# turian/inverse-audio-synthesis

Measured on AMD Instinct MI355X. Metric: audio-seconds rendered+lossed/sec (whole node), batch=128 4s@44.1kHz, higher is better.
Workload: dtype f32; 1 GPU; BASELINE configs[1]: torchsynth-style Voice render + PQMF(3) analysis + mel-L1 loss, batch 128 x 4 s @ 44100 Hz per GPU; batch_per_gpu=128, samples_per_voice=176400, launch=hipgraph, streams=5, pipelined=True

## Files before the change

inverse-audio-synthesis_amd/csrc/voice_ctrl_kernels.hip:

```cpp
#define IAS_CTL_NO_LIBM
#include "voice_math.h"
#include "wave_ops.h"
#include "voice_table.h"

#define CS_THREADS 256
#define CS_WAVES (CS_THREADS / 64)
#define CS_KERNEL __global__ __launch_bounds__(CS_THREADS) __attribute__((amdgpu_num_vgpr(28)))

__constant__ IasParamRange c_cs_table[IAS_NPARAMS] = IAS_PARAM_TABLE_INIT;
__device__ const double g_cs_tab[IAS_CTL_TAB_DOUBLES] = IAS_CTL_TAB_INIT;

__device__ __forceinline__ void cs_stage_table(double* s_tab) {
  for (int i = threadIdx.x; i < IAS_CTL_TAB_DOUBLES; i += CS_THREADS) s_tab[i] = g_cs_tab[i];
}
__device__ __forceinline__ float cs_mapped(const float* __restrict__ params01, int b, int idx, const double* s_tab) {
  const IasParamRange r = c_cs_table[idx];
  return ias_map_param(params01[(size_t)b * IAS_NPARAMS + idx], (float)r.lo, (float)r.span, (float)r.curve, r.symmetric, s_tab);
}
__device__ __forceinline__ int cs_adsr_base(int a) {
  switch (a) {
    case 0: return IAS_P_ADSR_1_ATTACK;
    case 1: return IAS_P_ADSR_2_ATTACK;
    case 2: return IAS_P_LFO_1_AMP_ADSR_ATTACK;
    case 3: return IAS_P_LFO_2_AMP_ADSR_ATTACK;
    case 4: return IAS_P_LFO_1_RATE_ADSR_ATTACK;
    default: return IAS_P_LFO_2_RATE_ADSR_ATTACK;
  }
}

CS_KERNEL void voice_env_slim_kernel(const float* __restrict__ params01, float* __restrict__ sig, int Tc, float control_rate) {
  __shared__ __attribute__((aligned(16))) double s_tab[IAS_CTL_TAB_DOUBLES];
  __shared__ float s_p[8];
  const int a = blockIdx.x, b = blockIdx.y, tid = threadIdx.x;
  cs_stage_table(s_tab);
  __syncthreads();
  if (tid < 5) s_p[tid] = cs_mapped(params01, b, cs_adsr_base(a) + tid, s_tab);
  if (tid == 5) s_p[5] = cs_mapped(params01, b, IAS_P_KEYBOARD_DURATION, s_tab);
  __syncthreads();
  IasAdsr e;
  e.attack = s_p[0]; e.decay = s_p[1]; e.sustain = s_p[2]; e.release = s_p[3]; e.alpha = s_p[4];
  const float note_on = s_p[5], eps = (float)IAS_EPS;
  if (tid == 0) s_p[6] = ias_adsr_heads(e, note_on, control_rate, eps, s_tab).decay_head;
  if (tid == 64) s_p[7] = ias_adsr_heads(e, note_on, control_rate, eps, s_tab).release_head;
  __syncthreads();
  IasAdsrHeads heads;
  heads.decay_head = s_p[6]; heads.release_head = s_p[7];
  float* out = sig + ((size_t)b * 8 + a) * Tc;
  for (int t = tid; t < Tc; t += CS_THREADS) out[t] = ias_adsr_headed(t, e, note_on, control_rate, eps, heads, s_tab);
}

CS_KERNEL void voice_lfo_slim_kernel(const float* __restrict__ params01, float* __restrict__ sig,
                                     float* __restrict__ dbg ,
                                     int Tc, float control_rate) {
  extern __shared__ __attribute__((aligned(16))) double cs_smem[];
  double* s_tab = cs_smem;
  double* s_sum = s_tab + IAS_CTL_TAB_DOUBLES;
  __shared__ double s_wtot[CS_WAVES];
  __shared__ float s_q[8];
  __shared__ float s_mode[8];
  const int l = blockIdx.x, b = blockIdx.y, tid = threadIdx.x, lane = tid & 63, wave = tid >> 6;
  const int qbase = (l == 0) ? IAS_P_LFO_1_FREQUENCY : IAS_P_LFO_2_FREQUENCY;
  cs_stage_table(s_tab);
  __syncthreads();
  if (tid < 8) s_q[tid] = cs_mapped(params01, b, qbase + tid, s_tab);
  __syncthreads();
  if (tid < 5) s_mode[tid] = ias_pow_ctl(s_q[3 + tid], IAS_LFO_EXPONENT_F, s_tab);
  const float freq = s_q[0], depth = s_q[1], phi = s_q[2];
  const float* rate_env = sig + ((size_t)b * 8 + 4 + l) * Tc;
  const float* amp_env = sig + ((size_t)b * 8 + 2 + l) * Tc;

  const int per_wave = ((Tc + CS_WAVES - 1) / CS_WAVES + 63) / 64 * 64;
  const int t_begin = min(wave * per_wave, Tc), t_end = min(t_begin + per_wave, Tc);
  double carry = 0.0;
  for (int t0 = t_begin; t0 < t_end; t0 += 64) {
    const int t = t0 + lane;
    double inc = 0.0;
    if (t < t_end) inc = (double)ias_lfo_inc(freq, depth, rate_env[t], control_rate);
    const double sc = wave_incl_scan(inc, lane) + carry;
    carry = __shfl(sc, 63, 64);
    if (t < t_end) s_sum[t] = sc;
  }
  if (lane == 0) s_wtot[wave] = carry;
  __syncthreads();
  double base = 0.0;
  for (int w = 0; w < wave; ++w) base += s_wtot[w];
  float mode[5];
  {
    const float sm = (float)((double)s_mode[0] + (double)s_mode[1] + (double)s_mode[2] + (double)s_mode[3] + (double)s_mode[4]);
#pragma unroll
    for (int k = 0; k < 5; ++k) mode[k] = ias_div(s_mode[k], sm);
  }
  float* out = sig + ((size_t)b * 8 + 6 + l) * Tc;
  for (int t = t_begin + lane; t < t_end; t += 64) {
    const double ph = base + s_sum[t];
    const float arg = ias_add((float)ph, phi);
    const float o = ias_mul(ias_lfo_shape_mix(arg, mode, s_tab), amp_env[t]);
    out[t] = o;
    if (dbg != nullptr) {
      dbg[((size_t)b * 10 + 6 + l) * Tc + t] = arg;
      dbg[((size_t)b * 10 + 8 + l) * Tc + t] = o;
    }
  }
}

CS_KERNEL void voice_modmix_slim_kernel(const float* __restrict__ params01, const float* __restrict__ sig,
                                        float* __restrict__ ctrl, IasVoiceConst* __restrict__ vconst,
                                        float* __restrict__ dbg, int Tc) {
  __shared__ __attribute__((aligned(16))) double s_tab[IAS_CTL_TAB_DOUBLES];
  __shared__ float s_w[20];
  __shared__ float s_p[IAS_NPARAMS];
  const int b = blockIdx.y, tid = threadIdx.x;
  cs_stage_table(s_tab);
  __syncthreads();
  if (tid < 20) s_w[tid] = cs_mapped(params01, b, IAS_P_MOD_MATRIX_ADSR_1_TO_VCO_1_PITCH + tid, s_tab);
  if (blockIdx.x == 0 && tid >= 64 && tid < 64 + IAS_NPARAMS) s_p[tid - 64] = cs_mapped(params01, b, tid - 64, s_tab);
  __syncthreads();
  const float* sb = sig + (size_t)b * 8 * Tc;
  const int t = blockIdx.x * CS_THREADS + tid;
  if (t < Tc) {
    const float e0 = sb[t], e1 = sb[Tc + t], l0 = sb[6 * Tc + t], l1 = sb[7 * Tc + t];
    float* out = ctrl + (size_t)b * IAS_NCTRL * Tc;
#pragma unroll
    for (int j = 0; j < IAS_NCTRL; ++j)
      out[j * Tc + t] = ias_dot4_cr(s_w[j], s_w[5 + j], s_w[10 + j], s_w[15 + j], e0, e1, l0, l1);
    if (dbg != nullptr) {
#pragma unroll
      for (int r = 0; r < 6; ++r) dbg[((size_t)b * 10 + r) * Tc + t] = sb[r * Tc + t];
    }
  }
  if (blockIdx.x == 0 && tid == 0) {
    const float* p = s_p;
    const float midi_f0 = p[IAS_P_KEYBOARD_MIDI_F0];
    IasVoiceConst vc;
    vc.f0_1 = ias_add(midi_f0, p[IAS_P_VCO_1_TUNING]);
    vc.depth_1 = p[IAS_P_VCO_1_MOD_DEPTH];
    vc.phi_1 = p[IAS_P_VCO_1_INITIAL_PHASE];
    vc.f0_2 = ias_add(midi_f0, p[IAS_P_VCO_2_TUNING]);
    vc.depth_2 = p[IAS_P_VCO_2_MOD_DEPTH];
    vc.phi_2 = p[IAS_P_VCO_2_INITIAL_PHASE];
    vc.kpart = ias_partials_k(midi_f0, vc.depth_2, s_tab);
    vc.shape = p[IAS_P_VCO_2_SHAPE];
    vc.shape_gain = ias_sub(1.0f, ias_div(vc.shape, 2.0f));
    vc.lvl0 = p[IAS_P_MIXER_VCO_1];
    vc.lvl1 = p[IAS_P_MIXER_VCO_2];
    vc.lvl2 = p[IAS_P_MIXER_NOISE];
    vc.pad[0] = vc.pad[1] = vc.pad[2] = vc.pad[3] = 0.0f;
    vconst[b] = vc;
  }
}

bool ias_voice_control_slim_ok(int Tc, int control_rate) {
  return Tc <= 4096 && (double)Tc / (double)control_rate <= 600.0;
}
int ias_voice_control_slim_launch(const float* params01, float* ctrl, void* vconst, float* sig, float* dbg, int B, int Tc,
                                  int control_rate, hipStream_t stream) {
  const size_t lds = sizeof(double) * (IAS_CTL_TAB_DOUBLES + (size_t)Tc);
  hipLaunchKernelGGL(voice_env_slim_kernel, dim3(6, B), dim3(CS_THREADS), 0, stream, params01, sig, Tc, (float)control_rate);
  hipLaunchKernelGGL(voice_lfo_slim_kernel, dim3(2, B), dim3(CS_THREADS), lds, stream, params01, sig, dbg, Tc, (float)control_rate);
  hipLaunchKernelGGL(voice_modmix_slim_kernel, dim3((Tc + CS_THREADS - 1) / CS_THREADS, B), dim3(CS_THREADS), 0, stream, params01,
                     (const float*)sig, ctrl, (IasVoiceConst*)vconst, dbg, Tc);
  return hipGetLastError() == hipSuccess ? IAS_OK : IAS_ERR_LAUNCH;
}
```

inverse-audio-synthesis_amd/csrc/voice_kernels.hip:

```cpp
#include <cstdio>
#include <cstdlib>
#include "voice_math.h"
#include "wave_ops.h"
#include "voice_trig.h"
#include "voice_table.h"

#define VOICE_THREADS 256
#define VOICE_WAVES (VOICE_THREADS / 64)
#define AUDIO_THREADS 256
#define AUDIO_WAVES (AUDIO_THREADS / 64)
#define VOICE_SPT 16
#define VOICE_TILE (AUDIO_THREADS * VOICE_SPT)

__constant__ IasParamRange c_param_table[IAS_NPARAMS] = IAS_PARAM_TABLE_INIT;


__device__ __forceinline__ float mapped_param(const float* __restrict__ params01, int b, int idx) {
  const IasParamRange r = c_param_table[idx];
  return ias_map_param(params01[(size_t)b * IAS_NPARAMS + idx], (float)r.lo, (float)r.span, (float)r.curve,
                       r.symmetric);
}

__device__ __forceinline__ int adsr_base(int a) {
  switch (a) {
// ... 436 lines not shown
      }
    }
    const float real = scale * (jf0 + (float)e);
    const float w1 = __builtin_amdgcn_fractf(real);
    voice_lds_cchar* cp = voice_ctrl_row(real, ctrl_biased);
    const voice_f2 qa = *(voice_lds_cfloat2*)(cp + 8), qb = *(voice_lds_cfloat2*)(cp + 24), qn = *(voice_lds_cfloat2*)(cp + 32);
    const float amp1 = fmaf(w1, qa.y, qa.x), amp2 = fmaf(w1, qb.y, qb.x), ampn = fmaf(w1, qn.y, qn.x);
    run1 += (double)inc1[e]; run2 += (double)inc2[e];
    const float arg1 = (float)run1 + vc.phi_1, arg2 = (float)run2 + vc.phi_2;
    float s2, c2, sgn;
    voice_sincos_sgn(arg2, s2, c2, sgn);
    const float th = voice_tanh_half_of_exp2arg(kexp * s2);
    const float v2 = th * fmaf(vc.shape, c2, sgn);
    float om = voice_cos(arg1) * amp1;
    om = fmaf(v2, amp2, om);
    om = fmaf(nz[e & 3], ampn, om);
    if (FAST || j0 + e < T) pk = fmaxf(pk, fabsf(om));
    o[e & 3] = om;
    if ((e & 3) == 3) {
      if (FAST) {
        *reinterpret_cast<float4*>(stage + lane * VOICE_SPT + 4 * ((e >> 2) ^ perm)) = make_float4(o[0], o[1], o[2], o[3]);
      } else {
        const int jq = j0 + e - 3;
#pragma unroll
        for (int x = 0; x < 4; ++x) if (jq + x < T) arow[jq + x] = o[x];
      }
      if ((e & (VOICE_GROUP - 1)) == VOICE_GROUP - 1) __builtin_amdgcn_sched_barrier(0);
    }
  }
  if (FAST) {
    const int dst = 4 * (lane ^ (lane >> 4));
#pragma unroll
    for (int q = 0; q < VOICE_SPT / 4; ++q)
      *reinterpret_cast<float4*>(arow + j_wave + q * 256 + dst) = *reinterpret_cast<const float4*>(stage + q * 256 + lane * 4);
  }
}

__device__ __forceinline__ float2 voice_ctrl_elem(const float* __restrict__ ctrl, const VoiceTile& t, int Tc, int i) {
  const int k = i / t.ncp, c = i - k * t.ncp;
  const float* crow = ctrl + ((size_t)t.b * IAS_NCTRL + k) * Tc;
  return make_float2(crow[t.c_lo + c], crow[min(t.c_lo + c + 1, Tc - 1)]);
}
__device__ __forceinline__ void voice_ctrl_put(char* dst, const VoiceTile& t, int i, float2 v, const IasVoiceConst& vc) {
  const int k = i / t.ncp, c = i - k * t.ncp;
  if (k == 1 || k == 3 || k == 4) {
    const float g = k == 1 ? vc.lvl0 : (k == 3 ? vc.lvl1 * vc.shape_gain : vc.lvl2);
    const float a = g * v.x;
    v = make_float2(a, g * v.y - a);
  }
  reinterpret_cast<float2*>(dst)[c * IAS_NCTRL + k] = v;
}

#define VOICE_WAVE_LOOKBACK (AUDIO_WAVES - 1)
#define VOICE_WAVE_PUBLISH (AUDIO_WAVES - 2)
template <int MATH, bool FMA_DIV>
__global__ __launch_bounds__(AUDIO_THREADS, VOICE_MIN_WAVES) __attribute__((amdgpu_num_vgpr(76))) void voice_audio_kernel(
    const float* __restrict__ ctrl, const IasVoiceConst* __restrict__ vconst,
    const float* __restrict__ noise, float* __restrict__ audio, unsigned long long* agg ,
    unsigned int* ticket_status ,
    unsigned* __restrict__ rowpeak, int T, int Tc, int ntiles, int nvoices, double inv_sample_rate, float sr_f,
    float sr_r, float scale, int maxctrl) {
  extern __shared__ __attribute__((aligned(16))) double dyn_smem_d[];
  double* s_tab = dyn_smem_d;
  float* s_stage = reinterpret_cast<float*>(dyn_smem_d + VOICE_TAB_DOUBLES);
  char* s_ctrl0 = reinterpret_cast<char*>(s_stage + VOICE_TILE);
  const int ctrl_bytes = maxctrl * VOICE_CTRL_ROW;
  __shared__ double s_wsum[2][2][AUDIO_WAVES];
  __shared__ double s_carry[2];
  __shared__ float s_max[AUDIO_WAVES];
  __shared__ int s_ticket;

  const int tid = threadIdx.x, lane = tid & 63, wave = tid >> 6;
  int my_counter = blockIdx.x % VOICE_NCOUNTERS, counters_tried = 0;
  if (tid == 0) s_ticket = voice_take_ticket(ticket_status, my_counter, counters_tried, ntiles, nvoices);
  if (MATH == VOICE_MATH_CR)
    for (int i = tid; i < IAS_EXP2_TAB_LEN; i += AUDIO_THREADS) s_tab[i] = g_exp2_tab[i];
  __syncthreads();

  VoiceTile cur = {}, next = {};
  bool have_cur = false;
  bool have_next = __builtin_amdgcn_readfirstlane(s_ticket) >= 0;
  float2 pre = make_float2(0.f, 0.f);
  if (have_next) {
    next = voice_tile_of(__builtin_amdgcn_readfirstlane(s_ticket), nvoices, T, Tc, scale);
    if (tid < IAS_NCTRL * next.ncp) pre = voice_ctrl_elem(ctrl, next, Tc, tid);
  }
  int slot = 0;
  float incC1[VOICE_SPT], incC2[VOICE_SPT];
  float incN1[VOICE_SPT], incN2[VOICE_SPT];
  double exC1 = 0.0, exC2 = 0.0, exN1 = 0.0, exN2 = 0.0;
#pragma unroll
  for (int e = 0; e < VOICE_SPT; ++e) { incC1[e] = incC2[e] = 0.0f; }

  while (have_cur || have_next) {
    gu64* row = (gu64*)(agg + ((size_t)cur.b * ntiles) * 2);
    VSTAMP(0);
    if (have_next) {
      char* dst = s_ctrl0 + (slot ^ 1) * ctrl_bytes;
      const IasVoiceConst vcp = vconst[next.b];
      if (tid < IAS_NCTRL * next.ncp) voice_ctrl_put(dst, next, tid, pre, vcp);
      for (int i = tid + AUDIO_THREADS; i < IAS_NCTRL * next.ncp; i += AUDIO_THREADS)
        voice_ctrl_put(dst, next, i, voice_ctrl_elem(ctrl, next, Tc, i), vcp);
    }
    unsigned long long early1 = VOICE_READY_BIT, early2 = VOICE_READY_BIT;
    if (have_cur) {
      if (wave == VOICE_WAVE_LOOKBACK && lane < cur.tile) {
        early1 = __hip_atomic_load(row + lane * 2, __ATOMIC_RELAXED, __HIP_MEMORY_SCOPE_AGENT);
        early2 = __hip_atomic_load(row + lane * 2 + 1, __ATOMIC_RELAXED, __HIP_MEMORY_SCOPE_AGENT);
      }
      if (cur.fast) {
        const int wave_u = __builtin_amdgcn_readfirstlane(wave);
        const float* nsrc = noise + (size_t)cur.b * T + cur.j_tile + wave_u * (64 * VOICE_SPT) + 4 * (lane ^ (lane >> 4));
#pragma unroll
        for (int q = 0; q < VOICE_SPT / 4; ++q)
          __builtin_amdgcn_global_load_lds((voice_glb_void*)(nsrc + q * 256),
                                           (voice_lds_void*)(s_stage + wave_u * (64 * VOICE_SPT) + q * 256), 16, 0, 0);
      }
    }
    __syncthreads();
    VSTAMP(1);
    unsigned after_raw = 0;
    int after_c = 0;
    if (have_next) {
      if (tid == 0) {
        after_c = my_counter;
        after_raw = __hip_atomic_fetch_add((gu32*)(ticket_status + after_c * 32), 1u, __ATOMIC_RELAXED, __HIP_MEMORY_SCOPE_AGENT);
      }
      const IasVoiceConst vcn = vconst[next.b];
#ifdef VOICE_SKIP_A
      if (false)
#else
      if (next.fast)
#endif
        voice_phase_a<MATH, FMA_DIV, true>(s_ctrl0 + (slot ^ 1) * ctrl_bytes, s_tab, vcn, next, T, inv_sample_rate, sr_f, sr_r,
                                           scale, incN1, incN2, exN1, exN2, s_wsum[slot ^ 1]);
#ifndef VOICE_ANALYZE_FULL_ONLY
      else
        voice_phase_a<MATH, FMA_DIV, false>(s_ctrl0 + (slot ^ 1) * ctrl_bytes, s_tab, vcn, next, T, inv_sample_rate, sr_f, sr_r,
                                            scale, incN1, incN2, exN1, exN2, s_wsum[slot ^ 1]);
#endif
      if (tid == 0) {
        const int nv_c = (nvoices - after_c + VOICE_NCOUNTERS - 1) / VOICE_NCOUNTERS;
        int tk = (after_c << 24) | (int)after_raw;
        if ((int)after_raw >= nv_c * ntiles) {
          my_counter = (my_counter + 1) % VOICE_NCOUNTERS;
          ++counters_tried;
          tk = voice_take_ticket(ticket_status, my_counter, counters_tried, ntiles, nvoices);
        }
        s_ticket = tk;
      }
    } else if (tid == 0) {
      s_ticket = -1;
    }
    VSTAMP(2);
    if (have_cur && wave == VOICE_WAVE_LOOKBACK) {
      double a1 = 0.0, a2 = 0.0;
      bool timeout = false;
      for (int t0 = 0; t0 < cur.tile; t0 += 64) {
        const int t = t0 + lane;
        unsigned long long x1 = VOICE_READY_BIT, x2 = VOICE_READY_BIT;
        if (t0 == 0) { x1 = early1; x2 = early2; }
        else if (t < cur.tile) { x1 = 0; x2 = 0; }
        unsigned spins = 0;
        bool ok = (x1 & x2 & VOICE_READY_BIT) != 0;
        while (!__all(ok)) {
          if (++spins > VOICE_SPIN_LIMIT) { timeout = true; break; }
          if (!ok) {
            x1 = __hip_atomic_load(row + t * 2, __ATOMIC_RELAXED, __HIP_MEMORY_SCOPE_AGENT);
            x2 = __hip_atomic_load(row + t * 2 + 1, __ATOMIC_RELAXED, __HIP_MEMORY_SCOPE_AGENT);
            ok = (x1 & x2 & VOICE_READY_BIT) != 0;
          }
          if (!__all(ok)) __builtin_amdgcn_s_sleep(VOICE_SPIN_SLEEP);
        }
        if (t < cur.tile) {
          a1 += __longlong_as_double((long long)(x1 & ~VOICE_READY_BIT));
          a2 += __longlong_as_double((long long)(x2 & ~VOICE_READY_BIT));
        }
      }
      a1 = wave_sum(a1); a2 = wave_sum(a2);
      if (lane == 0) {
        if (timeout) {
          a1 = a2 = __longlong_as_double(0x7ff8000000000000ll);
          __hip_atomic_store((gu32*)ticket_status + VOICE_NCOUNTERS * 32, 1u, __ATOMIC_RELAXED, __HIP_MEMORY_SCOPE_AGENT);
          __hip_atomic_store((gu32*)ticket_status - 32, 1u, __ATOMIC_RELAXED, __HIP_MEMORY_SCOPE_AGENT);
        }
        s_carry[0] = a1; s_carry[1] = a2;
      }
    }
    VSTAMP(3);
    __syncthreads();
    VSTAMP(4);
    if (have_next && wave == VOICE_WAVE_PUBLISH && lane < 2) {
      double a = 0.0;
      for (int w = 0; w < AUDIO_WAVES; ++w) a += s_wsum[slot ^ 1][lane][w];
      gu64* nrow_agg = (gu64*)(agg + ((size_t)next.b * ntiles) * 2);
      __hip_atomic_store(nrow_agg + next.tile * 2 + lane, (unsigned long long)__double_as_longlong(a) | VOICE_READY_BIT,
                         __ATOMIC_RELAXED, __HIP_MEMORY_SCOPE_AGENT);
    }
    const int t_after = __builtin_amdgcn_readfirstlane(s_ticket);
    const bool have_after = t_after >= 0;
    VoiceTile after = {};
    if (have_after) {
      after = voice_tile_of(t_after, nvoices, T, Tc, scale);
      if (tid < IAS_NCTRL * after.ncp) pre = voice_ctrl_elem(ctrl, after, Tc, tid);
    }
    if (have_cur) {
      const IasVoiceConst vc = vconst[cur.b];
      float pk = 0.0f;
#ifdef VOICE_SKIP_B
      if (false)
#else
      if (cur.fast)
#endif
        voice_phase_b<true>(s_ctrl0 + slot * ctrl_bytes, s_stage, vc, cur, noise + (size_t)cur.b * T, audio + (size_t)cur.b * T,
                            T, scale, incC1, incC2, exC1, exC2, s_carry, s_wsum[slot], pk);
#ifndef VOICE_ANALYZE_FULL_ONLY
      else
        voice_phase_b<false>(s_ctrl0 + slot * ctrl_bytes, s_stage, vc, cur, noise + (size_t)cur.b * T, audio + (size_t)cur.b * T,
                             T, scale, incC1, incC2, exC1, exC2, s_carry, s_wsum[slot], pk);
#endif
      pk = wave_max(pk);
      if (lane == 0) s_max[wave] = pk;
    }
    VSTAMP(5);
    __syncthreads();
    VSTAMP(6);
    if (have_cur && tid == 0) {
      float m = s_max[0];
      for (int w = 1; w < AUDIO_WAVES; ++w) m = fmaxf(m, s_max[w]);
      atomicMax(rowpeak + cur.b, __float_as_uint(m));
    }
    cur = next;
    have_cur = have_next;
    next = after;
    have_next = have_after;
    slot ^= 1;
#pragma unroll
    for (int e = 0; e < VOICE_SPT; ++e) { incC1[e] = incN1[e]; incC2[e] = incN2[e]; }
    exC1 = exN1; exC2 = exN2;
  }
}

__global__ __launch_bounds__(256) void voice_normalize_kernel(float* __restrict__ audio,
                                                              const unsigned* __restrict__ rowpeak,
                                                              int T, int nvec_per_row) {
  const int b = blockIdx.y;
  const float peak = __uint_as_float(rowpeak[b]);
  if (!(peak > 1.0f)) return;
  float* row = audio + (size_t)b * T;
  if ((T & 3) == 0) {
    float4* r4 = reinterpret_cast<float4*>(row);
    for (int i = blockIdx.x * blockDim.x + threadIdx.x; i < nvec_per_row; i += gridDim.x * blockDim.x) {
      float4 v = r4[i];
      v.x = ias_div(v.x, peak); v.y = ias_div(v.y, peak);
      v.z = ias_div(v.z, peak); v.w = ias_div(v.w, peak);
      r4[i] = v;
    }
  } else {
    for (int i = blockIdx.x * blockDim.x + threadIdx.x; i < T; i += gridDim.x * blockDim.x)
      row[i] = ias_div(row[i], peak);
  }
}

static inline size_t align_up(size_t x, size_t a) { return (x + a - 1) / a * a; }

struct VoiceWs {
  size_t off_ctrl, off_vconst, off_env, off_sticky, off_sync, sync_bytes, off_agg, off_peak, total;
  int ntiles;
};
static VoiceWs voice_ws_layout(int B, int T, int Tc) {
  VoiceWs w;
  w.ntiles = (T + VOICE_TILE - 1) / VOICE_TILE;
  size_t o = 0;
  w.off_ctrl = o;    o = align_up(o + sizeof(float) * (size_t)B * IAS_NCTRL * Tc, 256);
  w.off_vconst = o;  o = align_up(o + sizeof(IasVoiceConst) * (size_t)B, 256);
  w.off_env = o;     o = align_up(o + sizeof(float) * (size_t)B * 8 * Tc, 256);
  w.off_sticky = o;  o += 128;
  w.off_sync = o;
  w.off_agg = o + VOICE_SYNC_HEAD_BYTES;
  w.off_peak = w.off_agg + sizeof(unsigned long long) * (size_t)B * 2 * w.ntiles;
  w.sync_bytes = align_up(w.off_peak + sizeof(unsigned) * (size_t)B - w.off_sync, 16);
  o = align_up(w.off_sync + w.sync_bytes, 256);
  w.total = o;
  return w;
}

extern "C" long long ias_voice_workspace_bytes(int B, int T, int Tc) {
  if (B <= 0 || T <= 0 || Tc <= 1) return IAS_ERR_ARG;
  return (long long)voice_ws_layout(B, T, Tc).total;
}

static int voice_maxctrl(int T, int Tc) {
  return (int)((double)VOICE_TILE * (double)(Tc - 1) / (double)(T - 1)) + 6;
}

static int voice_check_dims(int B, int T, int Tc) {
  if (B <= 0 || T <= 1 || Tc <= 1 || B > 65535) return IAS_ERR_ARG;
  const double span = (double)VOICE_TILE * (double)(Tc - 1) / (double)(T - 1);
  if (span + 6.0 > (double)VOICE_MAXCTRL) return IAS_ERR_UNSUPPORTED;
  return IAS_OK;
}

bool ias_voice_control_slim_ok(int Tc, int control_rate);
int ias_voice_control_slim_launch(const float* params01, float* ctrl, void* vconst, float* sig, float* dbg, int B, int Tc,
                                  int control_rate, hipStream_t stream);

static int voice_control_launch(const float* params01, float* ctrl, void* vconst, float* sig, float* dbg, int B,
                                int Tc, int control_rate, void* stream_) {
  hipStream_t stream = (hipStream_t)stream_;
  if (!params01 || !ctrl || !vconst || !sig || B <= 0 || B > 65535 || Tc <= 1 || control_rate <= 0) return IAS_ERR_ARG;
  const char* form = ias_diag_env("IAS_VOICE_CTRL");
  if (form == nullptr && ias_voice_control_slim_ok(Tc, control_rate))
    return ias_voice_control_slim_launch(params01, ctrl, vconst, sig, dbg, B, Tc, control_rate, stream);
#ifdef IAS_DIAG
  const size_t flds = voice_control_fused_lds(Tc);
  if (flds <= 156 * 1024 && form != nullptr && form[0] == 'f') {
    static bool attr_set = false;
    if (!attr_set) {
      if (hipFuncSetAttribute((const void*)voice_control_fused_kernel, hipFuncAttributeMaxDynamicSharedMemorySize, 156 * 1024) != hipSuccess)
        return IAS_ERR_LAUNCH;
      attr_set = true;
    }
    hipLaunchKernelGGL(voice_control_fused_kernel, dim3(B), dim3(CTLF_THREADS), flds, stream, params01, sig, ctrl,
                       (IasVoiceConst*)vconst, dbg, Tc, (float)control_rate);
    return hipGetLastError() == hipSuccess ? IAS_OK : IAS_ERR_LAUNCH;
  }
#endif
  const size_t lds = sizeof(double) * (VOICE_WAVES + (size_t)Tc);
  if (lds > 160 * 1024) return IAS_ERR_UNSUPPORTED;
  hipLaunchKernelGGL(voice_env_kernel, dim3(6, B), dim3(VOICE_THREADS), 0, stream, params01, sig, Tc,
                     (float)control_rate);
  if (lds > 64 * 1024)
    (void)hipFuncSetAttribute((const void*)voice_lfo_kernel, hipFuncAttributeMaxDynamicSharedMemorySize, (int)lds);
  hipLaunchKernelGGL(voice_lfo_kernel, dim3(2, B), dim3(VOICE_THREADS), lds, stream, params01, sig, dbg, Tc,
                     (float)control_rate);
  hipLaunchKernelGGL(voice_modmix_kernel, dim3((Tc + VOICE_THREADS - 1) / VOICE_THREADS, B), dim3(VOICE_THREADS), 0,
                     stream, params01, sig, ctrl, (IasVoiceConst*)vconst, dbg, Tc);
  return hipGetLastError() == hipSuccess ? IAS_OK : IAS_ERR_LAUNCH;
}

extern "C" int ias_voice_control(const float* params01, float* ctrl, void* vconst, float* env, int B, int Tc,
                                 int control_rate, void* stream_) {
  return voice_control_launch(params01, ctrl, vconst, env, nullptr, B, Tc, control_rate, stream_);
}

extern "C" int ias_voice_control_ws(const float* params01, void* workspace, long long workspace_bytes, int B, int T,
                                    int Tc, int control_rate, void* stream_) {
  if (!workspace) return IAS_ERR_ARG;
  int rc = voice_check_dims(B, T, Tc);
  if (rc) return rc;
  const VoiceWs w = voice_ws_layout(B, T, Tc);
  if ((size_t)workspace_bytes < w.total) return IAS_ERR_WORKSPACE;
  char* ws = (char*)workspace;
  return voice_control_launch(params01, (float*)(ws + w.off_ctrl), ws + w.off_vconst, (float*)(ws + w.off_env), nullptr,
                              B, Tc, control_rate, stream_);
}

extern "C" int ias_voice_control_debug(const float* params01, float* ctrl, void* vconst, float* env, float* dbg,
                                       int B, int Tc, int control_rate, void* stream_) {
  if (!dbg) return IAS_ERR_ARG;
  return voice_control_launch(params01, ctrl, vconst, env, dbg, B, Tc, control_rate, stream_);
}

template <int MATH, bool FMA_DIV>
static int voice_audio_grid(size_t lds, int total_tiles) {
  static int cached_lds = -1, cached_grid = 0;
  if (cached_lds != (int)lds) {
    int dev = 0, ncu = 256, per_cu = 0;
    (void)hipGetDevice(&dev);
    (void)hipDeviceGetAttribute(&ncu, hipDeviceAttributeMultiprocessorCount, dev);
    if (hipOccupancyMaxActiveBlocksPerMultiprocessor(&per_cu, voice_audio_kernel<MATH, FMA_DIV>, AUDIO_THREADS, lds) != hipSuccess ||
        per_cu < 1)
      per_cu = 2;
    if (const char* e = ias_diag_env("IAS_VOICE_PERCU")) {
      const int v = atoi(e);
      if (v >= 1 && v < per_cu) per_cu = v;
    }
    cached_grid = per_cu * ncu;
    cached_lds = (int)lds;
    if (ias_diag_env("IAS_DEBUG")) fprintf(stderr, "[ias] voice_audio_kernel: %d workgroups/CU x %d CUs, %zu B LDS\n", per_cu, ncu, lds);
  }
  return cached_grid < total_tiles ? cached_grid : total_tiles;
}

template <int MATH, bool FMA_DIV>
static void voice_audio_launch(hipStream_t stream, const VoiceWs& w, char* ws, const float* noise, float* audio, int B,
                               int T, int Tc, int sample_rate) {
  const float scale = (float)(Tc - 1) / (float)(T - 1);
  const float sr_f = (float)sample_rate;
  const int maxctrl = voice_maxctrl(T, Tc);
  const size_t lds = sizeof(double) * VOICE_TAB_DOUBLES + sizeof(float) * VOICE_TILE + 2 * sizeof(float2) * IAS_NCTRL * (size_t)maxctrl;
  if (lds > 64 * 1024)
    (void)hipFuncSetAttribute((const void*)voice_audio_kernel<MATH, FMA_DIV>, hipFuncAttributeMaxDynamicSharedMemorySize, (int)lds);
  const int ntiles = w.ntiles;
  const int grid = voice_audio_grid<MATH, FMA_DIV>(lds, ntiles * B);
  hipLaunchKernelGGL((voice_audio_kernel<MATH, FMA_DIV>), dim3(grid), dim3(AUDIO_THREADS), lds, stream,
                     (const float*)(ws + w.off_ctrl), (const IasVoiceConst*)(ws + w.off_vconst), noise, audio,
                     (unsigned long long*)(ws + w.off_agg), (unsigned int*)(ws + w.off_sync),
                     (unsigned*)(ws + w.off_peak), T, Tc, ntiles, B, 1.0 / (double)sample_rate, sr_f,
                     1.0f / sr_f, scale, maxctrl);
}

extern "C" int ias_voice_stage(int stage, int math_mode, const float* noise, float* audio, void* workspace,
                               long long workspace_bytes, int B, int T, int Tc, int sample_rate, void* stream_) {
  hipStream_t stream = (hipStream_t)stream_;
  if (!workspace || sample_rate <= 0 || stage < 0 || stage > 3 || math_mode < 0 || math_mode > 1) return IAS_ERR_ARG;
  if (stage != 2 && (!noise || !audio)) return IAS_ERR_ARG;
  int rc = voice_check_dims(B, T, Tc);
  if (rc) return rc;
  const VoiceWs w = voice_ws_layout(B, T, Tc);
  if ((size_t)workspace_bytes < w.total) return IAS_ERR_WORKSPACE;
  char* ws = (char*)workspace;
  if (stage == 2) {
    if (hipMemsetAsync(ws + w.off_sync, 0, w.sync_bytes, stream) != hipSuccess) return IAS_ERR_LAUNCH;
  } else if (stage == 0 || stage == 3) {
    if (stage == 0 && hipMemsetAsync(ws + w.off_sync, 0, w.sync_bytes, stream) != hipSuccess) return IAS_ERR_LAUNCH;
    const bool fma_div = ias_div_fma_rate_ok(sample_rate) != 0;
    if (math_mode == VOICE_MATH_CR) {
      if (fma_div) voice_audio_launch<VOICE_MATH_CR, true>(stream, w, ws, noise, audio, B, T, Tc, sample_rate);
      else voice_audio_launch<VOICE_MATH_CR, false>(stream, w, ws, noise, audio, B, T, Tc, sample_rate);
    } else {
      if (fma_div) voice_audio_launch<VOICE_MATH_HW, true>(stream, w, ws, noise, audio, B, T, Tc, sample_rate);
      else voice_audio_launch<VOICE_MATH_HW, false>(stream, w, ws, noise, audio, B, T, Tc, sample_rate);
    }
  } else {
    const int nvec = T / 4;
    int gx = (nvec + 255) / 256;
    if (gx > 64) gx = 64;
    if (gx < 1) gx = 1;
    hipLaunchKernelGGL(voice_normalize_kernel, dim3(gx, B), dim3(256), 0, stream, audio, (unsigned*)(ws + w.off_peak), T,
                       nvec);
  }
  return hipGetLastError() == hipSuccess ? IAS_OK : IAS_ERR_LAUNCH;
}

extern "C" int ias_voice_render(const float* params01, const float* noise, float* audio, void* workspace,
                                long long workspace_bytes, int B, int T, int Tc, int sample_rate,
                                int control_rate, int normalize, int math_mode, void* stream_) {
  if (!params01 || !noise || !audio || !workspace || sample_rate <= 0 || control_rate <= 0) return IAS_ERR_ARG;
  int rc = voice_check_dims(B, T, Tc);
  if (rc) return rc;
  const VoiceWs w = voice_ws_layout(B, T, Tc);
  if ((size_t)workspace_bytes < w.total) return IAS_ERR_WORKSPACE;
  char* ws = (char*)workspace;
  rc = ias_voice_control(params01, (float*)(ws + w.off_ctrl), ws + w.off_vconst, (float*)(ws + w.off_env), B, Tc,
                         control_rate, stream_);
  for (int stage = 0; stage < (normalize ? 2 : 1) && rc == IAS_OK; ++stage)
    rc = ias_voice_stage(stage, math_mode, noise, audio, workspace, workspace_bytes, B, T, Tc, sample_rate, stream_);
  return rc;
}

extern "C" int ias_voice_read_status(const void* workspace, unsigned* status_dev, int B, int T, int Tc, void* stream_) {
  if (!workspace || !status_dev) return IAS_ERR_ARG;
  const VoiceWs w = voice_ws_layout(B, T, Tc);
  if (hipMemcpyAsync(status_dev, (const char*)workspace + w.off_sync + VOICE_NCOUNTERS * 128, sizeof(unsigned), hipMemcpyDeviceToDevice,
                     (hipStream_t)stream_) != hipSuccess)
    return IAS_ERR_LAUNCH;
  return IAS_OK;
}

extern "C" int ias_voice_read_status_sticky(void* workspace, unsigned* status_dev, int B, int T, int Tc, int clear,
                                            void* stream_) {
  if (!workspace || !status_dev) return IAS_ERR_ARG;
  const VoiceWs w = voice_ws_layout(B, T, Tc);
  char* word = (char*)workspace + w.off_sticky;
  if (hipMemcpyAsync(status_dev, word, sizeof(unsigned), hipMemcpyDeviceToDevice, (hipStream_t)stream_) != hipSuccess)
    return IAS_ERR_LAUNCH;
  if (clear && hipMemsetAsync(word, 0, sizeof(unsigned), (hipStream_t)stream_) != hipSuccess) return IAS_ERR_LAUNCH;
  return IAS_OK;
}

extern "C" long long ias_voice_ctrl_offset(int B, int T, int Tc) {
  if (B <= 0 || T <= 0 || Tc <= 1) return IAS_ERR_ARG;
  return (long long)voice_ws_layout(B, T, Tc).off_ctrl;
}
extern "C" long long ias_voice_vconst_offset(int B, int T, int Tc) {
  if (B <= 0 || T <= 0 || Tc <= 1) return IAS_ERR_ARG;
  return (long long)voice_ws_layout(B, T, Tc).off_vconst;
}

extern "C" long long ias_voice_peaks_offset(int B, int T, int Tc) {
  if (B <= 0 || T <= 0 || Tc <= 1) return IAS_ERR_ARG;
  return (long long)voice_ws_layout(B, T, Tc).off_peak;
}

__global__ __launch_bounds__(256) void voice_save_kernel(const float* __restrict__ ctrl, const float* __restrict__ vconst,
                                                         const float* __restrict__ peak, float* __restrict__ ctrl_out,
                                                         float* __restrict__ vconst_out, float* __restrict__ peaks_out,
                                                         long long nctrl, int nvc, int npk) {
  const long long i = (long long)blockIdx.x * 256 + threadIdx.x;
  if (i < nctrl) ctrl_out[i] = ctrl[i];
  if (i < nvc) vconst_out[i] = vconst[i];
  if (peaks_out && i < npk) peaks_out[i] = peak[i];
}
extern "C" int ias_voice_save_for_backward(const void* workspace, float* ctrl_out, float* vconst_out, float* peaks_out, int B,
                                           int T, int Tc, void* stream_) {
  if (!workspace || !ctrl_out || !vconst_out || B <= 0 || T <= 0 || Tc <= 1) return IAS_ERR_ARG;
  const VoiceWs w = voice_ws_layout(B, T, Tc);
  const char* ws = (const char*)workspace;
  const long long nctrl = (long long)B * IAS_NCTRL * Tc;
  static_assert(sizeof(IasVoiceConst) == 64, "vconst rows are 16 floats");
  const long long nthreads = nctrl > 16LL * B ? nctrl : 16LL * B;
  hipLaunchKernelGGL(voice_save_kernel, dim3((unsigned)((nthreads + 255) / 256)), dim3(256), 0, (hipStream_t)stream_,
                     (const float*)(ws + w.off_ctrl), (const float*)(ws + w.off_vconst), (const float*)(ws + w.off_peak),
                     ctrl_out, vconst_out, peaks_out, nctrl, B * 16, B);
  return hipGetLastError() == hipSuccess ? IAS_OK : IAS_ERR_LAUNCH;
}

extern "C" int ias_voice_read_peaks(const void* workspace, float* peaks_dev, int B, int T, int Tc, void* stream_) {
  if (!workspace || !peaks_dev) return IAS_ERR_ARG;
  const VoiceWs w = voice_ws_layout(B, T, Tc);
  if (hipMemcpyAsync(peaks_dev, (const char*)workspace + w.off_peak, sizeof(float) * (size_t)B,
                     hipMemcpyDeviceToDevice, (hipStream_t)stream_) != hipSuccess)
    return IAS_ERR_LAUNCH;
  return IAS_OK;
}
```

Measured before the change: 3.106 million audio-s/s.

## Fuse envelope, LFO and mod-matrix control kernels into one per-voice kernel

Replaces the three-kernel control path (ADSR envelopes, LFO scan, mod-matrix mix) with a single kernel per batch item that computes envelopes on the fly and keeps LFO outputs in shared memory. Intermediate envelope rows are written to global memory only when the caller needs them (the rows flag), so the render path skips those writes. This cuts two launches and the global round trip of the intermediate signal rows. The cost is only B blocks for the whole control stage, which lowers parallelism, plus some recomputation of envelopes. The old three-kernel path is kept behind a diagnostic flag.

```diff
diff --git a/inverse-audio-synthesis_amd/csrc/voice_ctrl_kernels.hip b/inverse-audio-synthesis_amd/csrc/voice_ctrl_kernels.hip
--- a/inverse-audio-synthesis_amd/csrc/voice_ctrl_kernels.hip
+++ b/inverse-audio-synthesis_amd/csrc/voice_ctrl_kernels.hip
@@ -28,6 +28,165 @@
   }
 }
 
+__device__ __forceinline__ float cs_uniform(float v) {
+  return __int_as_float(__builtin_amdgcn_readfirstlane(__float_as_int(v)));
+}
+
+__device__ __forceinline__ void cs_fence() { asm volatile("" ::: "memory"); }
+
+__device__ __forceinline__ float cs_env_at(int t, int a, const float* s_p, const float* s_head, float control_rate,
+                                           const double* s_tab) {
+  cs_fence();
+  const float* q = s_p + cs_adsr_base(a);
+  IasAdsr e;
+  e.attack = cs_uniform(q[0]); e.decay = cs_uniform(q[1]); e.sustain = cs_uniform(q[2]);
+  e.release = cs_uniform(q[3]); e.alpha = cs_uniform(q[4]);
+  IasAdsrHeads heads;
+  heads.decay_head = cs_uniform(s_head[2 * a]);
+  heads.release_head = cs_uniform(s_head[2 * a + 1]);
+  const float note_on = cs_uniform(s_p[IAS_P_KEYBOARD_DURATION]);
+  const float v = ias_adsr_headed(t, e, note_on, control_rate, (float)IAS_EPS, heads, s_tab);
+  cs_fence();
+  return v;
+}
+
+template <bool ROWS>
+CS_KERNEL void voice_ctrl_fused_slim_kernel(const float* __restrict__ params01, float* __restrict__ ctrl,
+                                            IasVoiceConst* __restrict__ vconst, float* __restrict__ sig ,
+                                            float* __restrict__ dbg , int Tc, float control_rate) {
+  extern __shared__ __attribute__((aligned(16))) double cs_smem[];
+  double* s_tab = cs_smem;
+  double* s_sum = s_tab + IAS_CTL_TAB_DOUBLES;
+  float* s_lfo = reinterpret_cast<float*>(s_sum + Tc);
+  __shared__ double s_wtot[2][CS_WAVES];
+  __shared__ float s_p[IAS_NPARAMS];
+  __shared__ float s_head[12];
+  __shared__ float s_mode[2][8];
+  const int b = blockIdx.x, tid = threadIdx.x, lane = tid & 63, wave = tid >> 6;
+  const float eps = (float)IAS_EPS;
+
+  cs_stage_table(s_tab);
+  __syncthreads();
+  if (tid < IAS_NPARAMS) s_p[tid] = cs_mapped(params01, b, tid, s_tab);
+  __syncthreads();
+  const float note_on = s_p[IAS_P_KEYBOARD_DURATION];
+  if (wave == 1) {
+    if (lane < 12) {
+      const float* q = s_p + cs_adsr_base(lane >> 1);
+      const float attack = q[0], decay = q[1], release = q[3], alpha = q[4];
+      const float new_attack = fminf(attack, note_on);
+      const float new_decay = fminf(fmaxf(ias_sub(note_on, attack), 0.0f), decay);
+      s_head[lane] = ias_ramp(0, (lane & 1) ? release : new_decay, (lane & 1) ? note_on : new_attack, 1, 1, alpha, control_rate,
+                              eps, s_tab);
+    }
+  } else if (wave == 2) {
+    if (lane < 16 && (lane & 7) < 5) {
+      const int qbase = (lane < 8) ? IAS_P_LFO_1_FREQUENCY : IAS_P_LFO_2_FREQUENCY;
+      s_mode[lane >> 3][lane & 7] = ias_pow_ctl(s_p[qbase + 3 + (lane & 7)], IAS_LFO_EXPONENT_F, s_tab);
+    }
+  } else if (wave == 3) {
+    if (lane == 0) {
+      const float* p = s_p;
+      const float midi_f0 = p[IAS_P_KEYBOARD_MIDI_F0];
+      IasVoiceConst vc;
+      vc.f0_1 = ias_add(midi_f0, p[IAS_P_VCO_1_TUNING]);
+      vc.depth_1 = p[IAS_P_VCO_1_MOD_DEPTH];
+      vc.phi_1 = p[IAS_P_VCO_1_INITIAL_PHASE];
+      vc.f0_2 = ias_add(midi_f0, p[IAS_P_VCO_2_TUNING]);
+      vc.depth_2 = p[IAS_P_VCO_2_MOD_DEPTH];
+      vc.phi_2 = p[IAS_P_VCO_2_INITIAL_PHASE];
+      vc.kpart = ias_partials_k(midi_f0, vc.depth_2, s_tab);
+      vc.shape = p[IAS_P_VCO_2_SHAPE];
+      vc.shape_gain = ias_sub(1.0f, ias_div(vc.shape, 2.0f));
+      vc.lvl0 = p[IAS_P_MIXER_VCO_1];
+      vc.lvl1 = p[IAS_P_MIXER_VCO_2];
+      vc.lvl2 = p[IAS_P_MIXER_NOISE];
+      vc.pad[0] = vc.pad[1] = vc.pad[2] = vc.pad[3] = 0.0f;
+      vconst[b] = vc;
+    }
+  }
+  __syncthreads();
+
+  if (tid == 0 || tid == 64) {
+    float* m = s_mode[wave];
+    const float sm = (float)((double)m[0] + (double)m[1] + (double)m[2] + (double)m[3] + (double)m[4]);
+    for (int k = 0; k < 5; ++k) m[k] = ias_div(m[k], sm);
+  }
+
+  const int per_wave = ((Tc + CS_WAVES - 1) / CS_WAVES + 63) / 64 * 64;
+  const int t_begin = min(wave * per_wave, Tc), t_end = min(t_begin + per_wave, Tc);
+  float* gsig = ROWS ? sig + (size_t)b * 8 * Tc : nullptr;
+  float* gdbg = (ROWS && dbg != nullptr) ? dbg + (size_t)b * 10 * Tc : nullptr;
+
+#pragma unroll 1
+  for (int l = 0; l < 2; ++l) {
+    const int qbase = (l == 0) ? IAS_P_LFO_1_FREQUENCY : IAS_P_LFO_2_FREQUENCY;
+    double carry = 0.0;
+    for (int t0 = t_begin; t0 < t_end; t0 += 64) {
+      const int t = t0 + lane;
+      double inc = 0.0;
+      if (t < t_end) {
+        const float r = cs_env_at(t, 4 + l, s_p, s_head, control_rate, s_tab);
+        inc = (double)ias_lfo_inc(cs_uniform(s_p[qbase]), cs_uniform(s_p[qbase + 1]), r, control_rate);
+        if (ROWS) {
+          gsig[(4 + l) * Tc + t] = r;
+          if (gdbg != nullptr) gdbg[(4 + l) * Tc + t] = r;
+        }
+      }
+      const double sc = wave_incl_scan(inc, lane) + carry;
+      carry = __shfl(sc, 63, 64);
+      if (t < t_end) s_sum[t] = sc;
+    }
+    if (lane == 0) s_wtot[l][wave] = carry;
+    __syncthreads();
+    for (int t = t_begin + lane; t < t_end; t += 64) {
+      float e0 = 0.0f, e1 = 0.0f;
+      if (l == 1) {
+        e0 = cs_env_at(t, 0, s_p, s_head, control_rate, s_tab);
+        e1 = cs_env_at(t, 1, s_p, s_head, control_rate, s_tab);
+      }
+      const float av = cs_env_at(t, 2 + l, s_p, s_head, control_rate, s_tab);
+      double base = 0.0;
+      for (int w = 0; w < wave; ++w) base += s_wtot[l][w];
+      const double ph = base + s_sum[t];
+      const float arg = ias_add((float)ph, cs_uniform(s_p[qbase + 2]));
+      float mode[5];
+#pragma unroll
+      for (int k = 0; k < 5; ++k) mode[k] = s_mode[l][k];
+      const float o = ias_mul(ias_lfo_shape_mix(arg, mode, s_tab), av);
+      cs_fence();
+      if (ROWS) {
+        gsig[(2 + l) * Tc + t] = av;
+        gsig[(6 + l) * Tc + t] = o;
+        if (gdbg != nullptr) {
+          gdbg[(2 + l) * Tc + t] = av;
+          gdbg[(6 + l) * Tc + t] = arg;
+          gdbg[(8 + l) * Tc + t] = o;
+        }
+      }
+      if (l == 0) {
+        s_lfo[t] = o;
+      } else {
+        const float l0 = s_lfo[t];
+        const float* s_w = s_p + IAS_P_MOD_MATRIX_ADSR_1_TO_VCO_1_PITCH;
+        float* out = ctrl + (size_t)b * IAS_NCTRL * Tc;
+#pragma unroll
+        for (int j = 0; j < IAS_NCTRL; ++j)
+          out[j * Tc + t] = ias_dot4_cr(s_w[j], s_w[5 + j], s_w[10 + j], s_w[15 + j], e0, e1, l0, o);
+        if (ROWS) {
+          gsig[t] = e0;
+          gsig[Tc + t] = e1;
+          if (gdbg != nullptr) {
+            gdbg[t] = e0;
+            gdbg[Tc + t] = e1;
+          }
+        }
+      }
+    }
+  }
+}
+
+#ifdef IAS_DIAG
 CS_KERNEL void voice_env_slim_kernel(const float* __restrict__ params01, float* __restrict__ sig, int Tc, float control_rate) {
   __shared__ __attribute__((aligned(16))) double s_tab[IAS_CTL_TAB_DOUBLES];
   __shared__ float s_p[8];
@@ -149,11 +308,8 @@
   }
 }
 
-bool ias_voice_control_slim_ok(int Tc, int control_rate) {
-  return Tc <= 4096 && (double)Tc / (double)control_rate <= 600.0;
-}
-int ias_voice_control_slim_launch(const float* params01, float* ctrl, void* vconst, float* sig, float* dbg, int B, int Tc,
-                                  int control_rate, hipStream_t stream) {
+int ias_voice_control_slim3_launch(const float* params01, float* ctrl, void* vconst, float* sig, float* dbg, int B, int Tc,
+                                   int control_rate, hipStream_t stream) {
   const size_t lds = sizeof(double) * (IAS_CTL_TAB_DOUBLES + (size_t)Tc);
   hipLaunchKernelGGL(voice_env_slim_kernel, dim3(6, B), dim3(CS_THREADS), 0, stream, params01, sig, Tc, (float)control_rate);
   hipLaunchKernelGGL(voice_lfo_slim_kernel, dim3(2, B), dim3(CS_THREADS), lds, stream, params01, sig, dbg, Tc, (float)control_rate);
@@ -161,3 +317,19 @@
                      (const float*)sig, ctrl, (IasVoiceConst*)vconst, dbg, Tc);
   return hipGetLastError() == hipSuccess ? IAS_OK : IAS_ERR_LAUNCH;
 }
+#endif
+
+bool ias_voice_control_slim_ok(int Tc, int control_rate) {
+  return Tc <= 4096 && (double)Tc / (double)control_rate <= 600.0;
+}
+int ias_voice_control_slim_launch(const float* params01, float* ctrl, void* vconst, float* sig, float* dbg, bool rows, int B,
+                                  int Tc, int control_rate, hipStream_t stream) {
+  const size_t lds = sizeof(double) * (IAS_CTL_TAB_DOUBLES + (size_t)Tc) + sizeof(float) * (size_t)Tc;
+  if (rows)
+    hipLaunchKernelGGL(voice_ctrl_fused_slim_kernel<true>, dim3(B), dim3(CS_THREADS), lds, stream, params01, ctrl,
+                       (IasVoiceConst*)vconst, sig, dbg, Tc, (float)control_rate);
+  else
+    hipLaunchKernelGGL(voice_ctrl_fused_slim_kernel<false>, dim3(B), dim3(CS_THREADS), lds, stream, params01, ctrl,
+                       (IasVoiceConst*)vconst, (float*)nullptr, (float*)nullptr, Tc, (float)control_rate);
+  return hipGetLastError() == hipSuccess ? IAS_OK : IAS_ERR_LAUNCH;
+}
diff --git a/inverse-audio-synthesis_amd/csrc/voice_kernels.hip b/inverse-audio-synthesis_amd/csrc/voice_kernels.hip
--- a/inverse-audio-synthesis_amd/csrc/voice_kernels.hip
+++ b/inverse-audio-synthesis_amd/csrc/voice_kernels.hip
@@ -762,17 +762,23 @@
 }
 
 bool ias_voice_control_slim_ok(int Tc, int control_rate);
-int ias_voice_control_slim_launch(const float* params01, float* ctrl, void* vconst, float* sig, float* dbg, int B, int Tc,
-                                  int control_rate, hipStream_t stream);
-
-static int voice_control_launch(const float* params01, float* ctrl, void* vconst, float* sig, float* dbg, int B,
+int ias_voice_control_slim_launch(const float* params01, float* ctrl, void* vconst, float* sig, float* dbg, bool rows, int B,
+                                  int Tc, int control_rate, hipStream_t stream);
+#ifdef IAS_DIAG
+int ias_voice_control_slim3_launch(const float* params01, float* ctrl, void* vconst, float* sig, float* dbg, int B, int Tc,
+                                   int control_rate, hipStream_t stream);
+#endif
+
+static int voice_control_launch(const float* params01, float* ctrl, void* vconst, float* sig, float* dbg, bool rows, int B,
                                 int Tc, int control_rate, void* stream_) {
   hipStream_t stream = (hipStream_t)stream_;
   if (!params01 || !ctrl || !vconst || !sig || B <= 0 || B > 65535 || Tc <= 1 || control_rate <= 0) return IAS_ERR_ARG;
   const char* form = ias_diag_env("IAS_VOICE_CTRL");
   if (form == nullptr && ias_voice_control_slim_ok(Tc, control_rate))
-    return ias_voice_control_slim_launch(params01, ctrl, vconst, sig, dbg, B, Tc, control_rate, stream);
+    return ias_voice_control_slim_launch(params01, ctrl, vconst, sig, dbg, rows, B, Tc, control_rate, stream);
 #ifdef IAS_DIAG
+  if (form != nullptr && form[0] == 's' && ias_voice_control_slim_ok(Tc, control_rate))
+    return ias_voice_control_slim3_launch(params01, ctrl, vconst, sig, dbg, B, Tc, control_rate, stream);
   const size_t flds = voice_control_fused_lds(Tc);
   if (flds <= 156 * 1024 && form != nullptr && form[0] == 'f') {
     static bool attr_set = false;
@@ -801,7 +807,7 @@
 
 extern "C" int ias_voice_control(const float* params01, float* ctrl, void* vconst, float* env, int B, int Tc,
                                  int control_rate, void* stream_) {
-  return voice_control_launch(params01, ctrl, vconst, env, nullptr, B, Tc, control_rate, stream_);
+  return voice_control_launch(params01, ctrl, vconst, env, nullptr, true, B, Tc, control_rate, stream_);
 }
 
 extern "C" int ias_voice_control_ws(const float* params01, void* workspace, long long workspace_bytes, int B, int T,
@@ -813,13 +819,13 @@
   if ((size_t)workspace_bytes < w.total) return IAS_ERR_WORKSPACE;
   char* ws = (char*)workspace;
   return voice_control_launch(params01, (float*)(ws + w.off_ctrl), ws + w.off_vconst, (float*)(ws + w.off_env), nullptr,
-                              B, Tc, control_rate, stream_);
+                              false, B, Tc, control_rate, stream_);
 }
 
 extern "C" int ias_voice_control_debug(const float* params01, float* ctrl, void* vconst, float* env, float* dbg,
                                        int B, int Tc, int control_rate, void* stream_) {
   if (!dbg) return IAS_ERR_ARG;
-  return voice_control_launch(params01, ctrl, vconst, env, dbg, B, Tc, control_rate, stream_);
+  return voice_control_launch(params01, ctrl, vconst, env, dbg, true, B, Tc, control_rate, stream_);
 }
 
 template <int MATH, bool FMA_DIV>
@@ -903,8 +909,8 @@
   const VoiceWs w = voice_ws_layout(B, T, Tc);
   if ((size_t)workspace_bytes < w.total) return IAS_ERR_WORKSPACE;
   char* ws = (char*)workspace;
-  rc = ias_voice_control(params01, (float*)(ws + w.off_ctrl), ws + w.off_vconst, (float*)(ws + w.off_env), B, Tc,
-                         control_rate, stream_);
+  rc = voice_control_launch(params01, (float*)(ws + w.off_ctrl), ws + w.off_vconst, (float*)(ws + w.off_env), nullptr, false,
+                            B, Tc, control_rate, stream_);
   for (int stage = 0; stage < (normalize ? 2 : 1) && rc == IAS_OK; ++stage)
     rc = ias_voice_stage(stage, math_mode, noise, audio, workspace, workspace_bytes, B, T, Tc, sample_rate, stream_);
   return rc;
```

Measured after the change: 3.127 million audio-s/s, median of 2. No clear change (+0.7%).
